# suilin0432/SoS-WSOD

Hardware: AMD Instinct MI355X
Metric: images/s (1/2/4/8 MI355X) VGG16+OICR 2000-prop; conv5_3 MFMA-util % (higher is better)
Workload: dtype bf16; 1 GPU; OICR+ training iteration: 4 views/step/GPU (1 image(s) x 2 scales x h-flip, every view 512x512), R=2000 proposals/view, K=20, VGG16 dilated-C5 + ROIPool 7x7 + fc6/fc7 4096 + WSDDN + 4 OICR heads, fwd+bwd+SGD(momentum, wd); image=one view, parallelism=dp1

## Files before the change

### include/soswsod_hip.h

```cpp
#ifndef SOSWSOD_HIP_H
#define SOSWSOD_HIP_H

#include <stdint.h>

#ifdef __cplusplus
extern "C" {
#endif

#ifndef SW_F32
#define SW_F32 0
#define SW_BF16 1
#endif

typedef struct ihipStream_t* sw_stream_t;

typedef struct sw_epilogue {
  const float* bias;
  int relu;
  const uint8_t* drop_mask;
  long ld_drop;
  float drop_scale;
  const void* relu_ref;
  long ld_ref;
  float ref_scale;
// ... 131 lines not shown
                        int32_t* out_classes, float* out_scores, int32_t* out_index, sw_stream_t stream);
typedef struct sw_stage_desc {
  const float* w;
  const float* bn_weight; const float* bn_bias; const float* bn_mean; const float* bn_var;
  float* scale; float* shift;
  void* dst;
  int32_t kind, rows, cols, block_start;
} sw_stage_desc;
int sw_stage_blocks(int kind, int rows, int cols);
int sw_stage_weights_multi(int dtype, int n, const sw_stage_desc* descs_dev, int total_blocks, float eps, sw_stream_t stream);
int sw_counter_add(uint64_t* counter, uint64_t increment, sw_stream_t stream);
typedef struct sw_copy_desc { const void* src; void* dst; long bytes; } sw_copy_desc;
int sw_copy_multi(int n, const sw_copy_desc* copies, sw_stream_t stream);
long sw_colsum_workspace_floats(int dtype, int M, int N);
int sw_colsum(int dtype, int M, int N, const void* X, long ld, float* out, float* workspace, int accumulate, sw_stream_t stream);
typedef struct { int M, N; const void* X; long ld; float* workspace; } sw_colsum_part_desc;
int sw_colsum_partial_multi(int dtype, int n, const sw_colsum_part_desc* parts, sw_stream_t stream);
typedef struct { int N, n_partial_rows; const float* workspace; float* out; } sw_colsum_fold_desc;
int sw_colsum_fold_multi(int n, const sw_colsum_fold_desc* folds, sw_stream_t stream);
int sw_convert_2d(int dtype, int rows, int cols, const float* src, long ld_src, void* dst, long ld_dst,
                  sw_stream_t stream);
int sw_split_bf16x3(int rows, int cols, const float* src, long ld_src, void* dst, long ld_dst, int side, int along_rows,
                    sw_stream_t stream);
int sw_convert_2d_t(int dtype, int rows, int cols, const float* src, long ld_src, void* dst, long ld_dst,
                    sw_stream_t stream);
int sw_nchw_to_nhwc(int dtype, int N, int C, int H, int W, int cpad, const float* in_nchw, void* out_nhwc,
                    sw_stream_t stream);
int sw_relu_bwd(int dtype, long n, const void* ref, const void* grad, void* out, sw_stream_t stream);
int sw_scale_cols(int dtype, int M, int N, const float* in, long ld_in, const float* colscale, void* out,
                  long ld_out, sw_stream_t stream);
// ... 201 lines not shown
```

### sos-wsod_amd/_lib.py

```python
import ctypes
import os

import torch

_HERE = os.path.dirname(os.path.abspath(__file__))
LIB_PATH = os.environ.get("SW_LIB_PATH") or os.path.join(_HERE, "libsoswsod_hip.so")

SW_F32, SW_BF16 = 0, 1

c_int, c_long, c_float, c_void_p, c_u64 = ctypes.c_int, ctypes.c_long, ctypes.c_float, ctypes.c_void_p, ctypes.c_uint64
c_int32, c_uint32, c_double, c_longlong = ctypes.c_int32, ctypes.c_uint32, ctypes.c_double, ctypes.c_longlong


class Epilogue(ctypes.Structure):
    _fields_ = [
        ("bias", c_void_p), ("relu", c_int), ("drop_mask", c_void_p), ("ld_drop", c_long), ("drop_scale", c_float),
        ("relu_ref", c_void_p), ("ld_ref", c_long), ("ref_scale", c_float), ("ref_dtype", c_int),
        ("out_dtype", c_int), ("accumulate_atomic", c_int), ("absmax_out", c_void_p),
        ("drop_seed", c_u64), ("drop_offset", c_u64), ("drop_hash_p", c_float), ("drop_offset_dev", c_void_p),
        ("splitk_workspace", c_void_p),
        ("residual", c_void_p), ("ld_res", c_long), ("res_dtype", c_int),
        ("fold_row_scale", c_void_p),
        ("sgd_fused", c_void_p), ("sgd_momentum", c_float), ("sgd_grad_scale", c_float),
    ]
# ... 116 lines not shown
                                   c_void_p, c_void_p, c_void_p, c_int, c_int, c_void_p, c_void_p, c_void_p]),
    "sw_oicr_update_boxes": (c_int, [c_int, c_int, c_int, c_int, c_int, c_void_p, c_long, c_int, c_int, c_void_p, c_void_p,
                                     c_void_p, _F4, c_float, c_void_p, c_void_p]),
    "sw_oicr_refine_loss": (c_int, [c_int, c_int, c_int, c_int, c_void_p, c_long, c_int, c_int, c_int, c_void_p, c_void_p,
                                    c_void_p, c_void_p, c_void_p, _F4, c_void_p, c_void_p, c_long, c_void_p,
                                    c_void_p, c_void_p, c_void_p]),
    "sw_oicr_predict": (c_int, [c_int, c_int, c_int, c_void_p, c_long, c_int, c_int, c_void_p, _F4, c_float, c_void_p,
                                c_void_p, c_void_p]),
    "sw_detect_workspace_bytes": (c_long, [c_int, c_int, c_int]),
    "sw_detect_postprocess": (c_int, [c_int, c_int, c_void_p, c_void_p, c_int, c_int, c_float, c_float, c_int, c_void_p,
                                      c_void_p, c_void_p, c_void_p, c_void_p, c_void_p, c_long, c_void_p]),
    "sw_tta_merge": (c_int, [c_int, c_int, c_int, c_void_p, c_void_p, c_void_p, c_void_p, c_void_p, c_int, c_int, c_float, c_int,
                             c_void_p, c_void_p, c_void_p, c_void_p, c_void_p, c_void_p]),
    "sw_colsum": (c_int, [c_int, c_int, c_int, c_void_p, c_long, c_void_p, c_void_p, c_int, c_void_p]),
    "sw_colsum_workspace_floats": (c_long, [c_int, c_int, c_int]),
    "sw_conv3x3_wgrad_small": (c_int, [c_int, c_int, c_int, c_int, c_int, c_int, c_void_p, c_void_p, c_void_p, c_void_p, c_int, c_void_p]),
    "sw_conv3x3_wgrad_fold": (c_int, [c_int, c_int, c_int, c_void_p, c_void_p, c_void_p, c_int, c_void_p]),
    "sw_conv3x3_wgrad_fold_multi": (c_int, [c_int, ctypes.POINTER(WgradFold), c_void_p]),
    "sw_conv3x3_multi": (c_int, [c_int, c_int, ctypes.POINTER(ConvProblem), c_void_p]),
    "sw_gemm_kk_grouped": (c_int, [c_int, c_int, ctypes.POINTER(GemmKKProblem), c_void_p]),
    "sw_gemm_kk_grouped_slabs": (c_long, [c_int, c_int, c_int]),
    "sw_splitk_fold_multi": (c_int, [c_int, ctypes.POINTER(SplitkFold), c_void_p]),
    "sw_colsum_fold_multi": (c_int, [c_int, ctypes.POINTER(ColsumFold), c_void_p]),
    "sw_colsum_partial_multi": (c_int, [c_int, c_int, ctypes.POINTER(ColsumPart), c_void_p]),
    "sw_conv3x3_wgrad_grouped": (c_int, [c_int, c_int, ctypes.POINTER(WgradProblem), c_void_p]),
    "sw_convert_2d": (c_int, [c_int, c_int, c_int, c_void_p, c_long, c_void_p, c_long, c_void_p]),
    "sw_split_bf16x3": (c_int, [c_int, c_int, c_void_p, c_long, c_void_p, c_long, c_int, c_int, c_void_p]),
    "sw_nchw_to_nhwc": (c_int, [c_int, c_int, c_int, c_int, c_int, c_int, c_void_p, c_void_p, c_void_p]),
    "sw_relu_bwd": (c_int, [c_int, c_long, c_void_p, c_void_p, c_void_p, c_void_p]),
    "sw_scale_cols": (c_int, [c_int, c_int, c_int, c_void_p, c_long, c_void_p, c_void_p, c_long, c_void_p]),
# ... 121 lines not shown
```

### sos-wsod_amd/backbone_vgg.py

```python
import os

import torch
import torch.nn as nn

from . import ops, staging, wgrad
from .registry import BACKBONE_REGISTRY
from .structures import ShapeSpec

_STAGES = [("plain1", 3, 64, 2), ("plain2", 64, 128, 2), ("plain3", 128, 256, 3), ("plain4", 256, 512, 3),
           ("plain5", 512, 512, 3)]


def _epc(dtype):
    return 8 if dtype == torch.bfloat16 else 4


class _Conv(nn.Module):

    def __init__(self, cin, cout):
        super().__init__()
        self.weight = nn.Parameter(torch.empty(cout, cin, 3, 3))
        self.bias = nn.Parameter(torch.zeros(cout))
        nn.init.kaiming_normal_(self.weight, mode="fan_out", nonlinearity="relu")

# ... 82 lines not shown
                pooled = torch.empty(cur.shape[0], oh, ow, cur.shape[3], device=x.device, dtype=dtype)
                ops.maxpool_fwd(cur, pooled, s)
                cur = pooled
            stage_info.append((conv_io, pre_pool))
        return cur, stage_info

    @staticmethod
    def backward(ctx, *gs):
        module, infos, params = ctx.module, ctx.infos, ctx.params
        ctx.infos = None
        n_in = len(infos)
        grads = [None] * len(params)
        first_trainable = module.first_trainable_conv()
        live = [i for i in range(n_in) if gs[i] is not None]
        if first_trainable is None or not live:
            return (None, None) + (None,) * n_in + tuple(grads)
        dev = gs[live[0]].device
        dtype = infos[0][0][0][0][0].dtype
        main = torch.cuda.current_stream()
        side = module.side_stream() if len(live) > 1 else None
        x3w = False
        if module.fp32x3 and dtype == torch.float32:
            x3w, pj = True, len(params)
            for sj in range(len(module.blocks) - 1, -1, -1):
                for cj in range(module.blocks[sj].num_conv - 1, -1, -1):
                    pj -= 2
                    if params[pj].requires_grad and not module.x3_layer(dtype, infos[live[0]][sj][0][cj][0].shape[3], module.blocks[sj].out_channels):
                        x3w = False
        wdt, nmul = (torch.bfloat16, 6) if x3w else (dtype, 1)
        bk = 64 if wdt == torch.bfloat16 else 32
# ... 40 lines not shown
                if (si, ci) == first_trainable:
                    break
            if si == first_trainable[0]:
                break
        if side is not None:
            side.wait_stream(main)
        for k, i in enumerate(live):
            st = side if (side is not None and k % 2 == 1) else main
            with torch.cuda.stream(st):
                g = gs[i]
                if st is not main:
                    g.record_stream(st)
                _VGGFunction._backward_one(module, infos[i], params, g, dtype, plan, i, first_trainable,
                                           deferred, None if st is main else main, x3w)
            infos[i] = None
        if side is not None:
            main.wait_stream(side)
        if deferred:
            ops.conv3x3_wgrad_grouped(deferred, tag="wgrad_grouped")
            ops.colsum_partial_multi(module._colsum_deferred)
            deferred.clear()
        module._colsum_deferred = []
        ops.conv3x3_wgrad_fold_multi([(pl["ws"], pl["nslab"], pl["dw"]) for pl in plan.values()])
        ops.colsum_fold_multi([(pl["rows"], pl["nrow"], pl["db"]) for pl in plan.values()])
        for pidx, pl in plan.items():
            w = params[pidx]
            grads[pidx] = pl["dw"][:, : w.shape[1]].contiguous() if pl["cin"] != w.shape[1] else pl["dw"]
            grads[pidx + 1] = pl["db"]
        return (None, None) + (None,) * n_in + tuple(grads)

    @staticmethod
    def _backward_one(module, stage_info, params, g, dtype, plan, i, first_trainable, deferred, consumer_stream, x3w=False):
        g = g.contiguous()
        if g.dtype != dtype:
            g = g.to(dtype)
        last_out = stage_info[-1][0][-1][1]
        assert stage_info[-1][1] is None, "backward expects the last stage to have no pool (vgg.py:197)"
        dz = ops.relu_bwd(last_out, g, out=torch.empty_like(g))
        pidx = len(params)
        for si in range(len(stage_info) - 1, -1, -1):
            blk = module.blocks[si]
            conv_io, _ = stage_info[si]
            for ci in range(blk.num_conv - 1, -1, -1):
                pidx -= 2
                x_in, _ = conv_io[ci]
                w = params[pidx]
                n, H, W, cin = x_in.shape
                pl = plan.get(pidx)
                if pl is not None:
                    npix = n * H * W
                    xw, dw_ = x_in, dz
                    if x3w:
                        cout = blk.out_channels
# ... 164 lines not shown
```

### sos-wsod_amd/csrc/elementwise.hip

```cpp
#include "common.h"
#include "soswsod_hip.h"

namespace {

inline int grid_for(long n, int block = 256) {
  long g = (n + block - 1) / block;
  return (int)(g < 1 ? 1 : (g > 2048 ? 2048 : g));
}

template <typename T>
__global__ void preprocess_kernel(int H, int W, int cpad, const uint8_t* __restrict__ img, float m0, float m1, float m2,
                                  float s0, float s1, float s2, T* __restrict__ out) {
  const long npix = (long)H * W;
  for (long p = blockIdx.x * (long)blockDim.x + threadIdx.x; p < npix; p += (long)gridDim.x * blockDim.x) {
    const float v0 = __fdiv_rn((float)img[p] - m0, s0);
    const float v1 = __fdiv_rn((float)img[npix + p] - m1, s1);
    const float v2 = __fdiv_rn((float)img[2 * npix + p] - m2, s2);
    T* o = out + p * cpad;
    Elem<T>::store(o + 0, v0); Elem<T>::store(o + 1, v1); Elem<T>::store(o + 2, v2);
    for (int c = 3; c < cpad; ++c) Elem<T>::store(o + c, 0.f);
  }
}

constexpr int PRE_MAX = 16;
// ... 353 lines not shown

constexpr int CFOLD_MAX = 32;
struct ColsumFoldMulti {
  int n;
  int first_wg[CFOLD_MAX + 1];
  int N[CFOLD_MAX], rows[CFOLD_MAX];
  const float* ws[CFOLD_MAX];
  float* out[CFOLD_MAX];
};
__global__ __launch_bounds__(256) void colsum_fold_multi_kernel(ColsumFoldMulti f) {
  int wg;
  const int i = batch_find(f.first_wg, f.n, (int)blockIdx.x, &wg);
  colsum_fold_body(f.N[i], f.rows[i], f.ws[i], f.out[i], wg);
}

__global__ void dropout_mask_kernel(uint8_t* __restrict__ keep, long n, uint64_t seed, uint64_t offset, float p) {
  for (long i = blockIdx.x * (long)blockDim.x + threadIdx.x; i < n; i += (long)gridDim.x * blockDim.x) {
    keep[i] = dropout_uniform(sw_splitmix64(seed) + offset, (uint64_t)i) >= p ? 1 : 0;
  }
}

__global__ void sgd_kernel(float* __restrict__ p, const float* __restrict__ g, float* __restrict__ buf, long n, float lr,
                           float mom, float wd, int first, float gscale) {
  for (long i = blockIdx.x * (long)blockDim.x + threadIdx.x; i < n; i += (long)gridDim.x * blockDim.x) {
    const SgdWM u = sgd_update(p[i], g[i], buf[i], first, mom, gscale, lr, wd);
    buf[i] = u.m;
    p[i] = u.w;
  }
}

// ... 26 lines not shown
  const float w1 = sgd_elem(d, j, h, mom, gscale);
  if (d.stage_kind) { if (d.stage_dtype == SW_BF16) sgd_stage<unsigned short>(d, j, w1); else sgd_stage<float>(d, j, w1); }
}
__device__ __forceinline__ void sgd_update4(float* w, const float4 g4, float* buf, int first, float mom, float gscale, SgdHyper h) {
  const float4 m4 = *(const float4*)buf;
  const float g[4] = {g4.x, g4.y, g4.z, g4.w};
  float m[4] = {m4.x, m4.y, m4.z, m4.w};
#pragma unroll
  for (int e = 0; e < 4; ++e) {
    const SgdWM u = sgd_update(w[e], g[e], m[e], first, mom, gscale, h.lr, h.wd);
    m[e] = u.m; w[e] = u.w;
  }
  *(float4*)buf = make_float4(m[0], m[1], m[2], m[3]);
}

__host__ __device__ __forceinline__ bool sgd_conv_tileable(const sw_sgd_tensor& d) {
  return d.stage_kind == 2 && (d.d0 % 32) == 0 && (d.d1 % 32) == 0;
}

template <typename T>
__device__ __forceinline__ void sgd_conv_tile(const sw_sgd_tensor& d, int blk, float mom, float gscale, float (*tile)[289]) {
  const int cib = d.d1 / 32;
  const int co0 = (blk / cib) * 32, ci0 = (blk % cib) * 32;
  const int Cin = d.d1, Cout = d.d0;
  const SgdHyper h = sgd_hyper(d.hyper_dev, d.lr, d.weight_decay);
  for (int idx = threadIdx.x; idx < 32 * 288; idx += 256) {
    const int co_l = idx / 288, rem = idx - co_l * 288;
    tile[co_l][rem] = sgd_elem(d, ((long)(co0 + co_l) * Cin + ci0) * 9 + rem, h, mom, gscale);
  }
  __syncthreads();
  if (d.stage0) {
    T* s0 = (T*)d.stage0;
    for (int idx = threadIdx.x; idx < 32 * 288; idx += 256) {
      const int co_l = idx / 288, r2 = idx - co_l * 288;
      const int tap = r2 >> 5, ci_l = r2 & 31;
      Elem<T>::store(s0 + ((long)(co0 + co_l) * 9 + tap) * d.d2 + ci0 + ci_l, tile[co_l][ci_l * 9 + tap]);
    }
  }
  if (d.stage1) {
    T* s1 = (T*)d.stage1;
    for (int idx = threadIdx.x; idx < 32 * 288; idx += 256) {
      const int ci_l = idx / 288, r3 = idx - ci_l * 288;
      const int tapf = r3 >> 5, co_l = r3 & 31;
      Elem<T>::store(s1 + ((long)(ci0 + ci_l) * 9 + tapf) * Cout + co0 + co_l, tile[co_l][ci_l * 9 + (8 - tapf)]);
    }
  }
}

__global__ __launch_bounds__(256) void sgd_multi_kernel(SgdBatch b, float mom, float gscale) {
  __shared__ float conv_tile[32][289];
  int blk;
  const sw_sgd_tensor& d = b.t[batch_find(b.block_start, b.n, (int)blockIdx.x, &blk)];
  if (sgd_conv_tileable(d)) {
    if (d.stage_dtype == SW_BF16) sgd_conv_tile<unsigned short>(d, blk, mom, gscale, conv_tile);
    else sgd_conv_tile<float>(d, blk, mom, gscale, conv_tile);
    return;
  }
  const SgdHyper h = sgd_hyper(d.hyper_dev, d.lr, d.weight_decay);
  const long base = (long)blk * SGD_CHUNK;
  const long end = min(d.n, base + SGD_CHUNK);
  const bool vec = ((((uintptr_t)d.param) | ((uintptr_t)d.grad) | ((uintptr_t)d.momentum_buf)) & 15) == 0;
  if (vec) {
    for (long i = base + threadIdx.x * 4; i < end; i += 256 * 4) {
      if (i + 4 <= end) {
        const float4 w4 = *(const float4*)(d.param + i);
// ... 558 lines not shown
  }
  if (!accumulate) {
    hipError_t e = hipMemsetAsync(out, 0, (size_t)N * sizeof(float), stream);
    if (e != hipSuccess) return (int)e;
  }
  if (M <= 0) return 0;
  const int slabs = (N + 63) / 64;
  int chunks = (2048 + slabs - 1) / slabs;
  int rpc = (M + chunks - 1) / chunks;
  if (rpc < 32) rpc = 32;
  chunks = (M + rpc - 1) / rpc;
  dim3 grid(slabs, chunks);
  DISPATCH_T(dtype,
    hipLaunchKernelGGL(colsum_kernel<unsigned short>, grid, dim3(256), 0, stream, M, N, rpc, (const unsigned short*)X, ld, out),
    hipLaunchKernelGGL(colsum_kernel<float>, grid, dim3(256), 0, stream, M, N, rpc, (const float*)X, ld, out));
  SW_CHECK_LAUNCH();
  return 0;
}

extern "C" int sw_fill_zero(void* p, long bytes, hipStream_t stream) {
  SW_ENTER();
  if (bytes <= 0) return 0;
  return (int)hipMemsetAsync(p, 0, (size_t)bytes, stream);
}

extern "C" int sw_dropout_mask(uint8_t* keep, long n, uint64_t seed, uint64_t offset, float p, hipStream_t stream) {
  SW_ENTER();
  if (n <= 0) return 0;
  hipLaunchKernelGGL(dropout_mask_kernel, dim3(grid_for(n)), dim3(256), 0, stream, keep, n, seed, offset, p);
  SW_CHECK_LAUNCH();
// ... 53 lines not shown
        dim3 grid(d.d0 / 64, (unsigned)(rows / 64));
        if (d.stage_dtype == SW_BF16)
          hipLaunchKernelGGL(sgd_tile_t_kernel<unsigned short>, grid, dim3(256), 0, stream, (int)rows, d.d0, d.param, d.grad,
                             d.momentum_buf, (long)d.d0, d.lr, d.weight_decay, d.first_step, momentum, grad_scale,
                             (unsigned short*)d.stage0, d.ld0, (unsigned short*)d.stage1, d.ld1, d.hyper_dev);
        else
          hipLaunchKernelGGL(sgd_tile_t_kernel<float>, grid, dim3(256), 0, stream, (int)rows, d.d0, d.param, d.grad,
                             d.momentum_buf, (long)d.d0, d.lr, d.weight_decay, d.first_step, momentum, grad_scale,
                             (float*)d.stage0, d.ld0, (float*)d.stage1, d.ld1, d.hyper_dev);
        SW_CHECK_LAUNCH();
        continue;
      }
      if (d.stage_kind && d.stage_dtype != SW_BF16 && d.stage_dtype != SW_F32) return -1;
      if (d.stage_kind == 1 && (d.d0 <= 0 || d.stage0 == nullptr)) return -5;
      if (d.stage_kind == 2 && (long)d.d0 * d.d1 * 9 != d.n) return -5;
      const long nb = sgd_conv_tileable(d) ? (long)(d.d0 / 32) * (d.d1 / 32) : (d.n + SGD_CHUNK - 1) / SGD_CHUNK;
      if (nb > (1L << 30)) return -6;
      b.t[t.n] = d;
      if (!t.add(nb)) return -6;
    }
    b.n = t.n;
    if (b.n == 0) continue;
    hipLaunchKernelGGL(sgd_multi_kernel, dim3((unsigned)t.blocks), dim3(256), 0, stream, b, momentum, grad_scale);
    SW_CHECK_LAUNCH();
  }
  return 0;
}

extern "C" int sw_mean_views(int V, long n, const float* in, float* out, hipStream_t stream) {
  SW_ENTER();
  if (n <= 0) return 0;
// ... 289 lines not shown
```

### sos-wsod_amd/ops.py

```python
import ctypes

import torch

from ._lib import SW_BF16, SW_F32, Epilogue, check, lib


def _p(t):
    return None if t is None else ctypes.c_void_p(t.data_ptr())


def _floats(vals, n):
    return (ctypes.c_float * n)(*[float(v) for v in vals])


def _workspace256(nbytes, device):
    ws = torch.empty(nbytes + 256, device=device, dtype=torch.uint8)
    return ws, ctypes.c_void_p((ws.data_ptr() + 255) // 256 * 256)


_raw_stream = getattr(torch._C, "_cuda_getCurrentRawStream", None)


def _stream():
    if _raw_stream is not None:
# ... 528 lines not shown
    rw = _floats(reg_weights, 4)
    if workspace is None:
        workspace = torch.empty(n_rounds * 2 * V * R, device=logits.device, dtype=torch.float32)
    assert tgt_box0 is None or (tgt_box0.dtype == torch.float32 and tgt_box0.is_contiguous() and tgt_box0.numel() == n_rounds * R * 4)
    check(lib.sw_oicr_refine_loss(V, R, K, n_rounds, _p(logits), logits.stride(0), cls_col, box_col, col_stride, _p(boxes),
                                  _p(lab_class), _p(lab_weight), _p(lab_index), _p(pred_view), rw, _p(loss_view),
                                  _p(dlogits), 0 if dlogits is None else dlogits.stride(0), _p(grad_scale), _p(workspace),
                                  _p(tgt_box0), _stream()), "sw_oicr_refine_loss")


def colsum(X, M, N, out, ld=None, accumulate=False):
    need = int(lib.sw_colsum_workspace_floats(dt(X), M, N))
    ws = torch.empty(max(need, 4), device=X.device, dtype=torch.float32)
    check(lib.sw_colsum(dt(X), M, N, _p(X), X.stride(0) if ld is None else ld, _p(out), _p(ws), int(accumulate), _stream()), "sw_colsum")
    return out


def convert_2d(src_f32, dst, rows, cols, ld_src=None, ld_dst=None):
    check(lib.sw_convert_2d(dt(dst), rows, cols, _p(src_f32), src_f32.stride(0) if ld_src is None else ld_src, _p(dst),
                            dst.stride(0) if ld_dst is None else ld_dst, _stream()), "sw_convert_2d")
    return dst


def split_bf16x3(src_f32, side, along_rows=False, out=None):
    _need_gpu(src_f32)
    rows, cols = src_f32.shape
    assert src_f32.dtype == torch.float32 and src_f32.stride(1) == 1
    shape = (6 * rows, cols) if along_rows else (rows, 6 * cols)
    if out is None or tuple(out.shape) != shape:
        out = torch.empty(shape[0], shape[1] + 128, device=src_f32.device, dtype=torch.bfloat16)[:, :shape[1]]
# ... 297 lines not shown


def nchw_to_nhwc(x_nchw_f32, out_nhwc):
    N, C, H, W = x_nchw_f32.shape
    check(lib.sw_nchw_to_nhwc(dt(out_nhwc), N, C, H, W, out_nhwc.shape[3], _p(x_nchw_f32), _p(out_nhwc), _stream()),
          "sw_nchw_to_nhwc")
    return out_nhwc


def relu_bwd(ref, grad, out=None):
    out = grad if out is None else out
    check(lib.sw_relu_bwd(dt(grad), grad.numel(), _p(ref), _p(grad), _p(out), _stream()), "sw_relu_bwd")
    return out


def scale_cols(src_f32, colscale, dst, M, N):
    check(lib.sw_scale_cols(dt(dst), M, N, _p(src_f32), src_f32.stride(0), _p(colscale), _p(dst), dst.stride(0), _stream()),
          "sw_scale_cols")
    return dst


def oicr_predict(logits, R, K, refine_k, base_col, round_stride, boxes, reg_weights, scale_clamp, all_scores, all_boxes):
    rw = _floats(reg_weights, 4)
    check(lib.sw_oicr_predict(R, K, refine_k, _p(logits), logits.stride(0), base_col, round_stride, _p(boxes), rw,
                              float(scale_clamp), _p(all_scores), _p(all_boxes), _stream()), "sw_oicr_predict")


def detect_postprocess(all_scores, all_boxes, img_h, img_w, score_thresh, nms_thresh, topk, out=None):
    R, K1 = all_scores.shape
    K = K1 - 1
# ... 539 lines not shown
```

### sos-wsod_amd/roi_heads_oicrplus.py

```python
from typing import Dict, List

import os
import numpy as np
import torch
import torch.nn as nn

from . import ops, staging
from .backbone_vgg import _dtype_from_cfg
from .box_head import DiscriminativeAdaptionNeck
from .events import get_event_storage, has_event_storage
from .fast_rcnn_oicr import OICROutputLayers
from .fast_rcnn_wsddn import WSDDNOutputLayers
from .inference import SCALE_CLAMP
from .poolers import ROIPooler
from .registry import ROI_BOX_HEAD_REGISTRY, ROI_HEADS_REGISTRY
from .structures import ShapeSpec

LOSS_NAMES_FMT = ["loss_cls"]


def get_image_level_gt(targets, num_classes):
    if targets is None:
        return None, None, None
    cls, ints, ohs = [], [], []
    for t in targets:
        g = t.gt_classes
        u = np.unique(g.detach().cpu().numpy().astype(np.int64))
        oh = np.zeros((1, num_classes), np.float32)
        oh[0, u] = 1.0
        cls.append(torch.from_numpy(u)); ints.append(torch.from_numpy(u)); ohs.append(torch.from_numpy(oh))
    return cls, ints, torch.cat(ohs, dim=0)


def _padded(rows, cols, device, dtype, pad=128):
    return torch.empty(rows, cols + pad, device=device, dtype=dtype)[:, :cols]


class LossDict(dict):

    def __init__(self, names, vector, total=None, finite=None):
        super().__init__({n: vector[i] for i, n in enumerate(names)})
        self.vector = vector
        self._total, self._finite = total, finite

    def total(self):
        return self.vector.sum() if self._total is None else self._total.view(())

    def finite_flag(self):
        return None if self._finite is None else self._finite.view(())

# ... 455 lines not shown
            g_losses = g_losses.contiguous().float()
        if g_total is not None:
            g_total = g_total.contiguous().float()
        dl = torch.empty(M, LD, device=dev, dtype=dt_)
        ops.scale_cols_loss(st["dlogits"], g_losses, g_total, self._c2l, 1.0 / B, dl, M, LD, self.n_head_cols)
        rs = 2.0 if st["train_dropout"] else 1.0
        dbh = torch.empty(LD, device=dev, dtype=torch.float32); ops.colsum(dl, M, LD, dbh)
        dWh = torch.empty(LD, D2, device=dev, dtype=torch.float32)
        ops.gemm(dl, h2, dWh, LD, D2, M, a_kstrided=True, b_kstrided=True, splitk=4)
        dz2 = _padded(M, D2, dev, dt_)
        WhT = self._head_weights_t(Wh, dev)
        if WhT is not None:
            ops.gemm(dl, WhT, dz2, M, D2, LD, ep=ops.make_epilogue(relu_ref=h2, ref_scale=rs, out_dtype=dt_))
        else:
            ops.gemm(dl, Wh, dz2, M, D2, LD, b_kstrided=True, ep=ops.make_epilogue(relu_ref=h2, ref_scale=rs, out_dtype=dt_))
        db2 = ops.grad_target(self.box_head.fc2.bias, (D2,), dev); ops.colsum(dz2, M, D2, db2)
        epc = 8 if dt_ == torch.bfloat16 else 4
        wgrad_nn = M % epc == 0

        def dz_t(dz, D):
            return ops.transpose_2d(dz, torch.empty(D, M + 8 * epc, device=dev, dtype=dt_)[:, :M], M, D)
        dW2 = ops.grad_target(self.box_head.fc2.weight, (D2, D1), dev)
        if wgrad_nn:
            self._fc_gemm(dz_t(dz2, D2), h1, dW2, D2, D1, M, b_kstrided=True)
        else:
            ops.gemm(dz2, h1, dW2, D2, D1, M, a_kstrided=True, b_kstrided=True)
        dz1 = _padded(M, D1, dev, dt_)
        if st.get("W2T") is not None:
            self._fc_gemm(dz2, st["W2T"], dz1, M, D1, D2, ep=ops.make_epilogue(relu_ref=h1, ref_scale=rs, out_dtype=dt_),
                          wname="fc2T", wmaster=self.box_head.fc2.weight)
        else:
            ops.gemm(dz2, W2, dz1, M, D1, D2, b_kstrided=True, ep=ops.make_epilogue(relu_ref=h1, ref_scale=rs, out_dtype=dt_))
        st["dz1"] = dz1
        dparams = [dW2, db2]
        row = 0
        for i in range(2, len(params_top), 2):
            n = params_top[i].shape[0]
            dparams += [dWh[row:row + n], dbh[row:row + n]]
            row += n
        return [g if p.requires_grad else None for g, p in zip(dparams, params_top)]

    def _fused_fc1_plan(self, M, D0, D1):
        opt = getattr(self, "_fused_opt", None)
        if (opt is None or self.compute_dtype != torch.bfloat16 or (M % 8) or getattr(self, "fp32x3", False)
                or getattr(self, "_fc6_panels", None) is not None or getattr(self, "_staged", False)
                or not ops.gemm_sgd_fused_supported(torch.bfloat16, D1, D0, M, False, True)):
            return None
        w = self.box_head.fc1.weight
        if not w.requires_grad or w.grad is not None:
            return None
        return opt.fused_update_entry(w)

    def _fused_fc1_wgrad(self, st):
        plan = st.pop("fused_fc1")
        entry, momentum, finish = plan
        pooled, dz1 = st["pooled"], st["dz1"]
        dev, M = pooled.device, st["inp"]["M"]
        D0, D1 = pooled.shape[1], dz1.shape[1]

        def nn():
            dzt = ops.transpose_2d(dz1, torch.empty(D1, M + 64, device=dev, dtype=torch.bfloat16)[:, :M], M, D1)
            scratch = torch.empty(D1, D0, device=dev, dtype=torch.float32)
            ep = ops.attach_sgd_fused(ops.make_epilogue(out_dtype=torch.float32), entry, momentum, 1.0)
            ops.gemm(dzt, pooled, scratch, D1, D0, M, b_kstrided=True, ep=ep)
        ops._launch("fc6_wgrad_sgd", nn)
        finish()

    def _train_backward_fc6(self, st, defer_fused=False):
        dt_ = self.compute_dtype
        pooled, dz1 = st["pooled"], st["dz1"]
        dev, M = pooled.device, st["inp"]["M"]
        D0, D1 = pooled.shape[1], dz1.shape[1]
        epc = 8 if dt_ == torch.bfloat16 else 4
        db1 = ops.grad_target(self.box_head.fc1.bias, (D1,), dev); ops.colsum(dz1, M, D1, db1)
        plan = self._fused_fc1_plan(M, D0, D1)
        if plan is not None:
            st["fused_fc1"] = plan
            if not defer_fused:
                self._fused_fc1_wgrad(st)
            return None, db1
        dW1 = ops.grad_target(self.box_head.fc1.weight, (D1, D0), dev)
        panels = getattr(self, "_fc6_panels", None)
        if panels is not None and panels[0] > 1 and D1 % (256 * panels[0]) == 0:
            rows = D1 // panels[0]
            dzt = ops.transpose_2d(dz1, torch.empty(D1, M + 8 * epc, device=dev, dtype=dt_)[:, :M], M, D1) if M % epc == 0 else None
            for i in range(panels[0]):
                if dzt is not None:
                    ops.gemm(dzt[i * rows:(i + 1) * rows], pooled, dW1[i * rows:(i + 1) * rows], rows, D0, M, b_kstrided=True)
                else:
                    ops.gemm(dz1[:, i * rows:(i + 1) * rows], pooled, dW1[i * rows:(i + 1) * rows], rows, D0, M, a_kstrided=True, b_kstrided=True)
                panels[1](i, dW1[i * rows:(i + 1) * rows])
        elif M % epc == 0:
            def nn():
                dzt = ops.transpose_2d(dz1, torch.empty(D1, M + 8 * epc, device=dev, dtype=dt_)[:, :M], M, D1)
                self._fc_gemm(dzt, pooled, dW1, D1, D0, M, b_kstrided=True)
            ops._launch("fc6_wgrad", nn)
        else:
            ops.gemm(dz1, pooled, dW1, D1, D0, M, a_kstrided=True, b_kstrided=True, tag="fc6_wgrad")
        return dW1, db1

    def _train_backward_pool(self, st, feat_req):
        dt_ = self.compute_dtype
        inp = st["inp"]
        B, Rs, offs, M = inp["B"], inp["R"], inp["off"], inp["M"]
        pooled, dz1, W1 = st["pooled"], st["dz1"], st["W1"]
        dev = pooled.device
        D0, D1 = pooled.shape[1], dz1.shape[1]
        dfeats = [None] * len(feat_req)
        if any(feat_req):
            dpooled = _padded(M, D0, dev, dt_, pad=64)
# ... 4 lines not shown
            else:
                ops.gemm(dz1, W1, dpooled, M, D0, D1, b_kstrided=True, ep=ops.make_epilogue(out_dtype=dt_, absmax_out=amax),
                         tag="fc6_dgrad")
            P = self.box_pooler.output_size
            for b in range(B):
                R, off = Rs[b], offs[b]
                for s in range(2):
                    if not feat_req[2 * b + s]:
                        continue
                    f = st["feats"][2 * b + s]
                    df = torch.empty_like(f)
                    r0 = off + 2 * s * R
                    ops.roi_pool_bwd(dpooled[r0:r0 + 2 * R], st["argmax"][r0:r0 + 2 * R], inp["rois"][b][s], df, P, P,
                                     row_scale=inp["obj"][b][2 * s:2 * s + 2].reshape(-1), row_scale_add=1.0, relu_ref=f,
                                     dout_absmax=amax, tag="roi_bwd", spatial_scale=self.box_pooler.scale)
                    dfeats[2 * b + s] = df
        if "fused_fc1" in st:
            self._fused_fc1_wgrad(st)
        return dfeats

    def _prepare_inputs(self, proposals_list, targets1, device, need_grad):
        K = self.num_classes
        B = len(proposals_list[0])
        assert B >= 1 and all(len(p) == B for p in proposals_list)
        _, gt_ints, gt_oh = get_image_level_gt(targets1, K)
        if not hasattr(self, "_consts") or self._consts[0].device != device:
            self._consts = (torch.ones(max(2, 2 * self.refine_K), device=device),
                            torch.tensor([0, 1, 2, 2], dtype=torch.int32, device=device),
                            torch.tensor([1, -1, 1, -1], dtype=torch.int32, device=device))
        Rs, Gs, offs, boxes, obj, rois = [], [], [], [], [], []
# ... 90 lines not shown
```

Measured before the change: 500.3 images/s.

## Fuse dz colsum with transpose, skip redundant ReLU bwd, vectorize SGD conv tiles

Adds a dz_side kernel that computes the bias-gradient column sum while writing the transposed dz for the fc6/fc7 wgrad GEMMs, replacing separate colsum and transpose passes over the same data. The ROI-pool backward, which already applies the ReLU mask via relu_ref, now marks its output so the backbone's final relu_bwd pass is skipped. The SGD conv-tile update is also vectorized with float4 loads/stores and a halved Cout tile. This saves several memory-bound passes but relies on a pointer-keyed registry to skip masking, which is fragile if buffers alias.

Result: no change. 501.7 images/s (median of 6 runs) (+0.3%).

```diff
diff --git a/include/soswsod_hip.h b/include/soswsod_hip.h
--- a/include/soswsod_hip.h
+++ b/include/soswsod_hip.h
@@ -169,6 +169,8 @@
 int sw_copy_multi(int n, const sw_copy_desc* copies, sw_stream_t stream);
 long sw_colsum_workspace_floats(int dtype, int M, int N);
 int sw_colsum(int dtype, int M, int N, const void* X, long ld, float* out, float* workspace, int accumulate, sw_stream_t stream);
+int sw_dz_side(int dtype, int M, int N, const void* X, long ld, void* XT, long ldt, float* out, float* workspace, int accumulate,
+               sw_stream_t stream);
 typedef struct { int M, N; const void* X; long ld; float* workspace; } sw_colsum_part_desc;
 int sw_colsum_partial_multi(int dtype, int n, const sw_colsum_part_desc* parts, sw_stream_t stream);
 typedef struct { int N, n_partial_rows; const float* workspace; float* out; } sw_colsum_fold_desc;
diff --git a/sos-wsod_amd/_lib.py b/sos-wsod_amd/_lib.py
--- a/sos-wsod_amd/_lib.py
+++ b/sos-wsod_amd/_lib.py
@@ -154,6 +154,7 @@
                              c_void_p, c_void_p, c_void_p, c_void_p, c_void_p, c_void_p]),
     "sw_colsum": (c_int, [c_int, c_int, c_int, c_void_p, c_long, c_void_p, c_void_p, c_int, c_void_p]),
     "sw_colsum_workspace_floats": (c_long, [c_int, c_int, c_int]),
+    "sw_dz_side": (c_int, [c_int, c_int, c_int, c_void_p, c_long, c_void_p, c_long, c_void_p, c_void_p, c_int, c_void_p]),
     "sw_conv3x3_wgrad_small": (c_int, [c_int, c_int, c_int, c_int, c_int, c_int, c_void_p, c_void_p, c_void_p, c_void_p, c_int, c_void_p]),
     "sw_conv3x3_wgrad_fold": (c_int, [c_int, c_int, c_int, c_void_p, c_void_p, c_void_p, c_int, c_void_p]),
     "sw_conv3x3_wgrad_fold_multi": (c_int, [c_int, ctypes.POINTER(WgradFold), c_void_p]),
diff --git a/sos-wsod_amd/backbone_vgg.py b/sos-wsod_amd/backbone_vgg.py
--- a/sos-wsod_amd/backbone_vgg.py
+++ b/sos-wsod_amd/backbone_vgg.py
@@ -120,6 +120,7 @@
         first_trainable = module.first_trainable_conv()
         live = [i for i in range(n_in) if gs[i] is not None]
         if first_trainable is None or not live:
+            ops.clear_relu_masked()
             return (None, None) + (None,) * n_in + tuple(grads)
         dev = gs[live[0]].device
         dtype = infos[0][0][0][0][0].dtype
@@ -190,6 +191,7 @@
                 _VGGFunction._backward_one(module, infos[i], params, g, dtype, plan, i, first_trainable,
                                            deferred, None if st is main else main, x3w)
             infos[i] = None
+        ops.clear_relu_masked()
         if side is not None:
             main.wait_stream(side)
         if deferred:
@@ -212,7 +214,10 @@
             g = g.to(dtype)
         last_out = stage_info[-1][0][-1][1]
         assert stage_info[-1][1] is None, "backward expects the last stage to have no pool (vgg.py:197)"
-        dz = ops.relu_bwd(last_out, g, out=torch.empty_like(g))
+        if ops.take_relu_masked(g, last_out):
+            dz = g
+        else:
+            dz = ops.relu_bwd(last_out, g, out=torch.empty_like(g))
         pidx = len(params)
         for si in range(len(stage_info) - 1, -1, -1):
             blk = module.blocks[si]
diff --git a/sos-wsod_amd/csrc/elementwise.hip b/sos-wsod_amd/csrc/elementwise.hip
--- a/sos-wsod_amd/csrc/elementwise.hip
+++ b/sos-wsod_amd/csrc/elementwise.hip
@@ -391,6 +391,94 @@
   colsum_fold_body(f.N[i], f.rows[i], f.ws[i], f.out[i], wg);
 }
 
+template <typename T>
+__device__ __forceinline__ void dz_side_load(u32x4 (&buf)[2], const T* __restrict__ src, long ld, bool cin, int row, int m0, int m1) {
+#pragma unroll
+  for (int s = 0; s < 2; ++s) {
+    const int m = row + 32 * s;
+    buf[s] = (cin && m >= m0 && m < m1) ? *(const u32x4*)(src + (long)m * ld) : u32x4{0u, 0u, 0u, 0u};
+  }
+}
+
+template <typename T>
+__global__ __launch_bounds__(256) void dz_side_kernel(int M, int N, int rows_per_chunk, const T* __restrict__ X, long ld,
+                                                      T* __restrict__ XT, long ldt, float* __restrict__ ws) {
+  constexpr int VEC = 16 / (int)sizeof(T), COLS = 8 * VEC, RP = 64 / VEC;
+  constexpr int NCH = COLS * 8 / 256;
+  __shared__ __attribute__((aligned(16))) T tile[2][COLS][64];
+  __shared__ float part[8][COLS + 4];
+  const int tid = threadIdx.x, col0 = blockIdx.x * COLS;
+  const int m0 = blockIdx.y * rows_per_chunk, m1 = min(M, m0 + rows_per_chunk);
+  const int A = m0 & ~(VEC - 1), off = m0 - A;
+  const int nt = (m1 - A + 63) / 64;
+  const int piece = tid & 7, lr0 = tid >> 3;
+  const bool cin = col0 + piece * VEC < N;
+  const T* src = X + col0 + piece * VEC;
+  const int sc = tid % COLS, rho0 = (tid / COLS) * NCH;
+  float acc[NCH];
+#pragma unroll
+  for (int n = 0; n < NCH; ++n) acc[n] = 0.f;
+  constexpr int G = 2;
+  u32x4 buf[G][2];
+  for (int tb = 0; tb < nt; tb += G) {
+#pragma unroll
+    for (int g = 0; g < G; ++g) dz_side_load<T>(buf[g], src, ld, cin, A + 64 * (tb + g) + lr0, m0, m1);
+#pragma unroll
+    for (int g = 0; g < G; ++g) {
+      const int t = tb + g;
+      if (t >= nt) break;
+      const u32x4 (&cur)[2] = buf[g];
+      T (*tl)[64] = tile[t & 1];
+#pragma unroll
+      for (int s = 0; s < 2; ++s) {
+        const int lr = lr0 + 32 * s, pr = (((lr >> 3) ^ piece) << 3) | (lr & 7);
+        const u32x4 x = cur[s];
+#pragma unroll
+        for (int v = 0; v < 4; ++v) {
+          if (sizeof(T) == 2) {
+            tl[piece * VEC + 2 * v][pr] = (T)(x[v] & 0xFFFFu);
+            tl[piece * VEC + 2 * v + 1][pr] = (T)(x[v] >> 16);
+          } else {
+            tl[piece * VEC + v][pr] = (T)__uint_as_float(x[v]);
+          }
+        }
+      }
+      __syncthreads();
+#pragma unroll
+      for (int k = 0; k < 8; ++k) {
+        const unsigned w = *(const unsigned*)&tl[sc][((k ^ ((sc / VEC) & 7)) << 3) | rho0];
+#pragma unroll
+        for (int n = 0; n < NCH; ++n) {
+          const int m = A + 64 * t + 8 * k + rho0 + n;
+          const float e = sizeof(T) == 2 ? __uint_as_float(n ? (w & 0xFFFF0000u) : (w << 16)) : __uint_as_float(w);
+          if (m >= m0 && m < m1) acc[n] += e;
+        }
+      }
+#pragma unroll
+      for (int s = 0; s < 2; ++s) {
+        const int i = tid + 256 * s, c = i / RP, rv = (i % RP) * VEC;
+        const int gc = col0 + c, gm = A + 64 * t + rv;
+        const int lo = max(m0, gm), hi = min(m1, gm + VEC);
+        if (gc >= N || lo >= hi) continue;
+        const T* p = &tl[c][(((rv >> 3) ^ ((c / VEC) & 7)) << 3) | (rv & 7)];
+        T* d = XT + (long)gc * ldt + gm;
+        if (hi - lo == VEC) *(u32x4*)d = *(const u32x4*)p;
+        else
+          for (int m = lo; m < hi; ++m) d[m - gm] = p[m - gm];
+      }
+    }
+  }
+#pragma unroll
+  for (int n = 0; n < NCH; ++n) part[(rho0 + n - off) & 7][sc] = acc[n];
+  __syncthreads();
+  if (tid < COLS && col0 + tid < N) {
+    float s = 0.f;
+#pragma unroll
+    for (int r = 0; r < 8; ++r) s += part[r][tid];
+    ws[(long)blockIdx.y * N + col0 + tid] = s;
+  }
+}
+
 __global__ void dropout_mask_kernel(uint8_t* __restrict__ keep, long n, uint64_t seed, uint64_t offset, float p) {
   for (long i = blockIdx.x * (long)blockDim.x + threadIdx.x; i < n; i += (long)gridDim.x * blockDim.x) {
     keep[i] = dropout_uniform(sw_splitmix64(seed) + offset, (uint64_t)i) >= p ? 1 : 0;
@@ -447,41 +535,70 @@
   *(float4*)buf = make_float4(m[0], m[1], m[2], m[3]);
 }
 
+constexpr int SGD_CONV_CO = 16, SGD_CONV_PITCH = 292;
 __host__ __device__ __forceinline__ bool sgd_conv_tileable(const sw_sgd_tensor& d) {
   return d.stage_kind == 2 && (d.d0 % 32) == 0 && (d.d1 % 32) == 0;
 }
 
 template <typename T>
-__device__ __forceinline__ void sgd_conv_tile(const sw_sgd_tensor& d, int blk, float mom, float gscale, float (*tile)[289]) {
+__device__ __forceinline__ void sgd_store4(T* o, float a, float b, float c, float e, bool vec) {
+  if (vec) {
+    if (sizeof(T) == 2) *(uint2*)o = make_uint2(pack_bf16x2(a, b), pack_bf16x2(c, e));
+    else *(float4*)o = make_float4(a, b, c, e);
+  } else {
+    Elem<T>::store(o, a); Elem<T>::store(o + 1, b); Elem<T>::store(o + 2, c); Elem<T>::store(o + 3, e);
+  }
+}
+
+template <typename T>
+__device__ __forceinline__ void sgd_conv_tile(const sw_sgd_tensor& d, int blk, float mom, float gscale, float (*tile)[SGD_CONV_PITCH]) {
+  constexpr int CO = SGD_CONV_CO, Q = CO / 4, P = SGD_CONV_PITCH;
   const int cib = d.d1 / 32;
-  const int co0 = (blk / cib) * 32, ci0 = (blk % cib) * 32;
+  const int co0 = (blk / cib) * CO, ci0 = (blk % cib) * 32;
   const int Cin = d.d1, Cout = d.d0;
   const SgdHyper h = sgd_hyper(d.hyper_dev, d.lr, d.weight_decay);
-  for (int idx = threadIdx.x; idx < 32 * 288; idx += 256) {
-    const int co_l = idx / 288, rem = idx - co_l * 288;
-    tile[co_l][rem] = sgd_elem(d, ((long)(co0 + co_l) * Cin + ci0) * 9 + rem, h, mom, gscale);
+  if (((((uintptr_t)d.param) | ((uintptr_t)d.grad) | ((uintptr_t)d.momentum_buf)) & 15) == 0) {
+    for (int idx = threadIdx.x; idx < CO * 72; idx += 256) {
+      const int co_l = idx / 72, f = idx - co_l * 72;
+      const long o = ((long)(co0 + co_l) * Cin + ci0) * 9 + 4 * f;
+      const float4 w4 = *(const float4*)(d.param + o);
+      float w[4] = {w4.x, w4.y, w4.z, w4.w};
+      sgd_update4(w, *(const float4*)(d.grad + o), d.momentum_buf + o, d.first_step, mom, gscale, h);
+      const float4 r = make_float4(w[0], w[1], w[2], w[3]);
+      *(float4*)(d.param + o) = r;
+      *(float4*)&tile[co_l][4 * f] = r;
+    }
+  } else {
+    for (int idx = threadIdx.x; idx < CO * 288; idx += 256) {
+      const int co_l = idx / 288, rem = idx - co_l * 288;
+      tile[co_l][rem] = sgd_elem(d, ((long)(co0 + co_l) * Cin + ci0) * 9 + rem, h, mom, gscale);
+    }
   }
   __syncthreads();
   if (d.stage0) {
     T* s0 = (T*)d.stage0;
-    for (int idx = threadIdx.x; idx < 32 * 288; idx += 256) {
-      const int co_l = idx / 288, r2 = idx - co_l * 288;
-      const int tap = r2 >> 5, ci_l = r2 & 31;
-      Elem<T>::store(s0 + ((long)(co0 + co_l) * 9 + tap) * d.d2 + ci0 + ci_l, tile[co_l][ci_l * 9 + tap]);
+    const bool vec = (d.d2 & 3) == 0 && (((uintptr_t)s0) & (4 * sizeof(T) - 1)) == 0;
+    for (int idx = threadIdx.x; idx < CO * 72; idx += 256) {
+      const int co_l = idx / 72, r2 = idx - co_l * 72;
+      const int tap = r2 >> 3, ci_l = (r2 & 7) * 4;
+      const float* t = &tile[co_l][ci_l * 9 + tap];
+      sgd_store4<T>(s0 + ((long)(co0 + co_l) * 9 + tap) * d.d2 + ci0 + ci_l, t[0], t[9], t[18], t[27], vec);
     }
   }
   if (d.stage1) {
     T* s1 = (T*)d.stage1;
-    for (int idx = threadIdx.x; idx < 32 * 288; idx += 256) {
-      const int ci_l = idx / 288, r3 = idx - ci_l * 288;
-      const int tapf = r3 >> 5, co_l = r3 & 31;
-      Elem<T>::store(s1 + ((long)(ci0 + ci_l) * 9 + tapf) * Cout + co0 + co_l, tile[co_l][ci_l * 9 + (8 - tapf)]);
+    const bool vec = (((uintptr_t)s1) & (4 * sizeof(T) - 1)) == 0;
+    for (int idx = threadIdx.x; idx < 32 * 9 * Q; idx += 256) {
+      const int ci_l = idx / (9 * Q), r3 = idx - ci_l * (9 * Q);
+      const int tapf = r3 / Q, co_l = (r3 - tapf * Q) * 4;
+      const float* t = &tile[co_l][ci_l * 9 + (8 - tapf)];
+      sgd_store4<T>(s1 + ((long)(ci0 + ci_l) * 9 + tapf) * Cout + co0 + co_l, t[0], t[P], t[2 * P], t[3 * P], vec);
     }
   }
 }
 
 __global__ __launch_bounds__(256) void sgd_multi_kernel(SgdBatch b, float mom, float gscale) {
-  __shared__ float conv_tile[32][289];
+  __shared__ __attribute__((aligned(16))) float conv_tile[SGD_CONV_CO][SGD_CONV_PITCH];
   int blk;
   const sw_sgd_tensor& d = b.t[batch_find(b.block_start, b.n, (int)blockIdx.x, &blk)];
   if (sgd_conv_tileable(d)) {
@@ -1070,6 +1187,25 @@
   DISPATCH_T(dtype,
     hipLaunchKernelGGL(colsum_kernel<unsigned short>, grid, dim3(256), 0, stream, M, N, rpc, (const unsigned short*)X, ld, out),
     hipLaunchKernelGGL(colsum_kernel<float>, grid, dim3(256), 0, stream, M, N, rpc, (const float*)X, ld, out));
+  SW_CHECK_LAUNCH();
+  return 0;
+}
+
+extern "C" int sw_dz_side(int dtype, int M, int N, const void* X, long ld, void* XT, long ldt, float* out, float* workspace,
+                          int accumulate, hipStream_t stream) {
+  SW_ENTER();
+  if (dtype != SW_BF16 && dtype != SW_F32) return -1;
+  const int vec = dtype == SW_BF16 ? 8 : 4;
+  if (!colsum_ws_ok(dtype, M, N, X, ld, workspace) || !XT || !out || ld < N || ldt < M || (ldt % vec) || (((uintptr_t)XT) & 15)) return -5;
+  int slabs, chunks, rpc;
+  colsum_ws_geometry(dtype, M, N, &slabs, &chunks, &rpc);
+  dim3 grid((N + 8 * vec - 1) / (8 * vec), chunks);
+  DISPATCH_T(dtype,
+    hipLaunchKernelGGL(dz_side_kernel<unsigned short>, grid, dim3(256), 0, stream, M, N, rpc, (const unsigned short*)X, ld,
+                       (unsigned short*)XT, ldt, workspace),
+    hipLaunchKernelGGL(dz_side_kernel<float>, grid, dim3(256), 0, stream, M, N, rpc, (const float*)X, ld, (float*)XT, ldt, workspace));
+  SW_CHECK_LAUNCH();
+  hipLaunchKernelGGL(colsum_fold_kernel, dim3((N + 15) / 16), dim3(256), 0, stream, N, chunks, workspace, out, accumulate);
   SW_CHECK_LAUNCH();
   return 0;
 }
@@ -1153,7 +1289,7 @@
       if (d.stage_kind && d.stage_dtype != SW_BF16 && d.stage_dtype != SW_F32) return -1;
       if (d.stage_kind == 1 && (d.d0 <= 0 || d.stage0 == nullptr)) return -5;
       if (d.stage_kind == 2 && (long)d.d0 * d.d1 * 9 != d.n) return -5;
-      const long nb = sgd_conv_tileable(d) ? (long)(d.d0 / 32) * (d.d1 / 32) : (d.n + SGD_CHUNK - 1) / SGD_CHUNK;
+      const long nb = sgd_conv_tileable(d) ? (long)(d.d0 / SGD_CONV_CO) * (d.d1 / 32) : (d.n + SGD_CHUNK - 1) / SGD_CHUNK;
       if (nb > (1L << 30)) return -6;
       b.t[t.n] = d;
       if (!t.add(nb)) return -6;
diff --git a/sos-wsod_amd/ops.py b/sos-wsod_amd/ops.py
--- a/sos-wsod_amd/ops.py
+++ b/sos-wsod_amd/ops.py
@@ -566,6 +566,17 @@
     ws = torch.empty(max(need, 4), device=X.device, dtype=torch.float32)
     check(lib.sw_colsum(dt(X), M, N, _p(X), X.stride(0) if ld is None else ld, _p(out), _p(ws), int(accumulate), _stream()), "sw_colsum")
     return out
+
+
+def dz_side(X, M, N, XT, out, accumulate=False, ws=None):
+    _need_gpu(X, XT, out)
+    if ws is None:
+        ws = torch.empty(max(int(lib.sw_colsum_workspace_floats(dt(X), M, N)), 4), device=X.device, dtype=torch.float32)
+    rc = lib.sw_dz_side(dt(X), M, N, _p(X), X.stride(0), _p(XT), XT.stride(0), _p(out), _p(ws), int(accumulate), _stream())
+    if rc == -5:
+        return False
+    check(rc, "sw_dz_side")
+    return True
 
 
 def convert_2d(src_f32, dst, rows, cols, ld_src=None, ld_dst=None):
@@ -893,6 +904,25 @@
     return out
 
 
+_relu_masked = set()
+
+
+def mark_relu_masked(grad, ref):
+    _relu_masked.add((grad.data_ptr(), ref.data_ptr(), grad.numel()))
+
+
+def take_relu_masked(grad, ref):
+    key = (grad.data_ptr(), ref.data_ptr(), grad.numel())
+    if key in _relu_masked:
+        _relu_masked.discard(key)
+        return True
+    return False
+
+
+def clear_relu_masked():
+    _relu_masked.clear()
+
+
 def scale_cols(src_f32, colscale, dst, M, N):
     check(lib.sw_scale_cols(dt(dst), M, N, _p(src_f32), src_f32.stride(0), _p(colscale), _p(dst), dst.stride(0), _stream()),
           "sw_scale_cols")
diff --git a/sos-wsod_amd/roi_heads_oicrplus.py b/sos-wsod_amd/roi_heads_oicrplus.py
--- a/sos-wsod_amd/roi_heads_oicrplus.py
+++ b/sos-wsod_amd/roi_heads_oicrplus.py
@@ -34,6 +34,14 @@
 
 def _padded(rows, cols, device, dtype, pad=128):
     return torch.empty(rows, cols + pad, device=device, dtype=dtype)[:, :cols]
+
+
+def _dz_side(dz, M, D, pitch, db):
+    dzt = torch.empty(D, pitch, device=dz.device, dtype=dz.dtype)[:, :M]
+    if not ops.dz_side(dz, M, D, dzt, db):
+        ops.colsum(dz, M, D, db)
+        ops.transpose_2d(dz, dzt, M, D)
+    return dzt
 
 
 class LossDict(dict):
@@ -519,16 +527,14 @@
             ops.gemm(dl, WhT, dz2, M, D2, LD, ep=ops.make_epilogue(relu_ref=h2, ref_scale=rs, out_dtype=dt_))
         else:
             ops.gemm(dl, Wh, dz2, M, D2, LD, b_kstrided=True, ep=ops.make_epilogue(relu_ref=h2, ref_scale=rs, out_dtype=dt_))
-        db2 = ops.grad_target(self.box_head.fc2.bias, (D2,), dev); ops.colsum(dz2, M, D2, db2)
+        db2 = ops.grad_target(self.box_head.fc2.bias, (D2,), dev)
         epc = 8 if dt_ == torch.bfloat16 else 4
         wgrad_nn = M % epc == 0
-
-        def dz_t(dz, D):
-            return ops.transpose_2d(dz, torch.empty(D, M + 8 * epc, device=dev, dtype=dt_)[:, :M], M, D)
         dW2 = ops.grad_target(self.box_head.fc2.weight, (D2, D1), dev)
         if wgrad_nn:
-            self._fc_gemm(dz_t(dz2, D2), h1, dW2, D2, D1, M, b_kstrided=True)
+            self._fc_gemm(_dz_side(dz2, M, D2, M + 8 * epc, db2), h1, dW2, D2, D1, M, b_kstrided=True)
         else:
+            ops.colsum(dz2, M, D2, db2)
             ops.gemm(dz2, h1, dW2, D2, D1, M, a_kstrided=True, b_kstrided=True)
         dz1 = _padded(M, D1, dev, dt_)
         if st.get("W2T") is not None:
@@ -556,7 +562,7 @@
             return None
         return opt.fused_update_entry(w)
 
-    def _fused_fc1_wgrad(self, st):
+    def _fused_fc1_wgrad(self, st, db1=None):
         plan = st.pop("fused_fc1")
         entry, momentum, finish = plan
         pooled, dz1 = st["pooled"], st["dz1"]
@@ -564,7 +570,9 @@
         D0, D1 = pooled.shape[1], dz1.shape[1]
 
         def nn():
-            dzt = ops.transpose_2d(dz1, torch.empty(D1, M + 64, device=dev, dtype=torch.bfloat16)[:, :M], M, D1)
+            dzt = st.pop("dz1t", None)
+            if dzt is None:
+                dzt = _dz_side(dz1, M, D1, M + 64, db1)
             scratch = torch.empty(D1, D0, device=dev, dtype=torch.float32)
             ep = ops.attach_sgd_fused(ops.make_epilogue(out_dtype=torch.float32), entry, momentum, 1.0)
             ops.gemm(dzt, pooled, scratch, D1, D0, M, b_kstrided=True, ep=ep)
@@ -577,16 +585,21 @@
         dev, M = pooled.device, st["inp"]["M"]
         D0, D1 = pooled.shape[1], dz1.shape[1]
         epc = 8 if dt_ == torch.bfloat16 else 4
-        db1 = ops.grad_target(self.box_head.fc1.bias, (D1,), dev); ops.colsum(dz1, M, D1, db1)
+        db1 = ops.grad_target(self.box_head.fc1.bias, (D1,), dev)
         plan = self._fused_fc1_plan(M, D0, D1)
         if plan is not None:
             st["fused_fc1"] = plan
             if not defer_fused:
-                self._fused_fc1_wgrad(st)
+                self._fused_fc1_wgrad(st, db1)
+            else:
+                st["dz1t"] = _dz_side(dz1, M, D1, M + 64, db1)
             return None, db1
         dW1 = ops.grad_target(self.box_head.fc1.weight, (D1, D0), dev)
         panels = getattr(self, "_fc6_panels", None)
-        if panels is not None and panels[0] > 1 and D1 % (256 * panels[0]) == 0:
+        in_panels = panels is not None and panels[0] > 1 and D1 % (256 * panels[0]) == 0
+        if in_panels or M % epc:
+            ops.colsum(dz1, M, D1, db1)
+        if in_panels:
             rows = D1 // panels[0]
             dzt = ops.transpose_2d(dz1, torch.empty(D1, M + 8 * epc, device=dev, dtype=dt_)[:, :M], M, D1) if M % epc == 0 else None
             for i in range(panels[0]):
@@ -597,8 +610,7 @@
                 panels[1](i, dW1[i * rows:(i + 1) * rows])
         elif M % epc == 0:
             def nn():
-                dzt = ops.transpose_2d(dz1, torch.empty(D1, M + 8 * epc, device=dev, dtype=dt_)[:, :M], M, D1)
-                self._fc_gemm(dzt, pooled, dW1, D1, D0, M, b_kstrided=True)
+                self._fc_gemm(_dz_side(dz1, M, D1, M + 8 * epc, db1), pooled, dW1, D1, D0, M, b_kstrided=True)
             ops._launch("fc6_wgrad", nn)
         else:
             ops.gemm(dz1, pooled, dW1, D1, D0, M, a_kstrided=True, b_kstrided=True, tag="fc6_wgrad")
@@ -633,6 +645,8 @@
                     ops.roi_pool_bwd(dpooled[r0:r0 + 2 * R], st["argmax"][r0:r0 + 2 * R], inp["rois"][b][s], df, P, P,
                                      row_scale=inp["obj"][b][2 * s:2 * s + 2].reshape(-1), row_scale_add=1.0, relu_ref=f,
                                      dout_absmax=amax, tag="roi_bwd", spatial_scale=self.box_pooler.scale)
+                    if getattr(self, "mark_masked_grad", True):
+                        ops.mark_relu_masked(df, f)
                     dfeats[2 * b + s] = df
         if "fused_fc1" in st:
             self._fused_fc1_wgrad(st)
```
